# Team766/ros_vision

Hardware: AMD Instinct MI355X
Metric: frames/sec + p50 per-frame latency, 1280x720 AprilTag detect at 1/2/4/8 MI355X (higher is better)
Workload: dtype u8

## Files before the change

ros_vision_amd/csrc/at_common.h:

```cpp
#pragma once

#include <hip/hip_runtime.h>
#include <stdint.h>

#include "at_detmath.h"

namespace at {

template <int TW>
struct CclTile {
  static constexpr int W = TW, H = 32;
  static constexpr int BW = TW / 2, BH = H / 2;
  static constexpr int NT = BW * BH;
  static constexpr int NODES = 3 * NT;
  static constexpr int ROW_NODES = 3 * BW;
};
constexpr int kCclTileH = 32;
constexpr int kCclTileNodesMax = CclTile<64>::NODES;
constexpr int kHashSlots = 4096;
constexpr int kHashBits = 12;
constexpr int kPairEntCap = 65536;
constexpr int kBndRows = 4;
constexpr int kBndPts = 64 * 4 * kBndRows * 4;
constexpr int kBndStage = 1024;
constexpr int kLdsPairSlots = 512;
constexpr uint32_t kTileNarrow = 0x80000000u;
constexpr int kMaxTilesPerFrame = 1024;
constexpr int kMaxCclTiles = 1024;
struct CclDesc {
  static constexpr int Tthr = 0, Bthr = 16, Lthr = 32, Rthr = 40;
  static constexpr int TsF = 48, TsL = 64, TsR = 80, BsF = 96, BsL = 112, BsR = 128;
  static constexpr int LsF = 144, LsL = 152, RsF = 160, RsR = 168;
  static constexpr int kWords = 176;
};
constexpr int kMergeCapMax = 15360;
constexpr int kMergeLdsMax = kMergeCapMax * 10;
constexpr int kMaxPairs = 4096;
constexpr int kSortCap = 8192;
constexpr int kBlobThreads = 256;
constexpr int kWideBlobMaxBatch = 8;
constexpr int kSmallBlob = 512;
constexpr int kNMaxima = 10;
constexpr int kMaxRefineSamples = 1536;
#ifndef AT_LDS_REFINE
#define AT_LDS_REFINE 256
#endif
constexpr int kLdsRefine = AT_LDS_REFINE;
constexpr int kDecodeGridPerBlobWg = 8;
inline int decode_grid(int nblobwg, int B) {
  const int hi = nblobwg * kDecodeGridPerBlobWg, want = 64 * B;
  return nblobwg * 2 > (want < hi ? want : hi) ? nblobwg * 2 : (want < hi ? want : hi);
}

constexpr int kNumStages = 12;
constexpr const char* kStageNames[kNumStages] = {"k_pre",   "k_thr_ccl", "k_ccl_merge", "k_ccl_roots",
                                                 "k_boundary", "k_pairs", "k_group",     "k_extents",
                                                 "k_blob_small", "k_blob", "k_decode",   "k_pose"};

constexpr int kNumCls = 7;
constexpr int kNumLargeCls = 3;

constexpr uint32_t kStatusPairsOverflow = 1u;
constexpr uint32_t kStatusHashFull = 2u;
constexpr uint32_t kStatusDetsOverflow = 4u;
constexpr uint32_t kStatusPointsOverflow = 8u;
constexpr uint32_t kStatusQuadsOverflow = 16u;
constexpr uint32_t kStatusPairsCapped = 32u;
constexpr int kMaxBatch = 256;
constexpr int kQcStride = 32;
constexpr int kQuadCandPerFrame = kMaxPairs;
constexpr int kMaxDets = kQuadCandPerFrame;
constexpr int kDetPoolPerFrame = 128;
constexpr int kMaxCodes = 1024;
constexpr int kMaxFamilyBits = 64;

struct FamilyDesc {
  int nbits;
  int width_at_border;
  int total_width;
  int reversed_border;
  int ncodes;
  int8_t bitx[kMaxFamilyBits], bity[kMaxFamilyBits];
};

struct Geom {
  int W, H, Wd, Hd;
  int TW, TH;
  int BW, BH;
  int CTX, CTY;
  int ctw;
  int merge_cap;
  int merge_lds;
  int nlarge;
  int bnd_region;
  int cap_pts;
  int BTX, BTY, ntb;
  uint32_t min_cluster;
  uint32_t max_cluster;
  int min_tag_width;
};

struct Params {
  int min_white_black_diff;
  float max_line_fit_mse;
  double cos_critical_rad;
  double decode_sharpening;
  int refine_edges;
  double fx, fy, cx, cy, k1, k2, p1, p2, k3;
  int diag_stop;
  double tag_size;
  int probe;
  int taps;
  int wide_blob;
  int pipe_stop;
  int lblob_wg;
  int sblob_wg;
  int dec_wg;
  FamilyDesc fam;
  int gp_w, gp_h, gp_c;
};
constexpr int kProbeWords = 256;

#ifdef AT_EXPERIMENTS
#define AT_DIAG_STOP(prm, n) ((prm).diag_stop == (n))
#define AT_PIPE_STOP(prm) ((prm).pipe_stop)
#define AT_PROBE_ON(prm) ((prm).probe != 0)
#define AT_DIAG_ANY(prm) ((prm).diag_stop != 0)
#else
#define AT_DIAG_STOP(prm, n) false
#define AT_PIPE_STOP(prm) 0
#define AT_PROBE_ON(prm) false
#define AT_DIAG_ANY(prm) false
#endif

struct KernelTimer {
  int stage;
  hipEvent_t t0, t1;
  hipError_t (*split)(void* ctx, int which);
  void* ctx;
};

struct DevDetection {
  int32_t id;
  int16_t hamming;
  uint16_t frame;
  float decision_margin;
  int32_t blob_rank;
  double H[9];
  double c[2];
  double p[4][2];
  double pose_R[9];
  double pose_t[3];
  double pose_err[2];
};

struct QuadCand {
  uint32_t frame, rank;
  float p[4][2];
};

struct QuadRecord {
  uint32_t blob_index, valid, accepted;
  uint16_t indices[4];
  float corners[4][2];
};

struct Moments {
  int32_t Mx, My, W;
  int64_t Mxx, Myy, Mxy;
  int32_t N;
};

struct QuadPend {
  float fit[4][4];
  uint32_t blob_index, valid;
  uint16_t indices[4];
};
static_assert(sizeof(QuadPend) == 80, "QuadPend: 80 B per kept blob");

struct DrawPrim {
  double x0, y0, x1, y1;
  uint8_t bgr[3];
};

struct DevBufs {
  const uint8_t* const* frames;
  uint8_t* gray;
  uint8_t* dec;
  uint8_t* mm;
  uint8_t* thr;
  uint32_t* par;
  uint32_t* lroot;
  uint32_t* nlroot;
  uint32_t* lcnt;
  uint32_t* cdesc;
  uint32_t* ccl_ovf;
  uint32_t* nlr_tot;
  uint32_t* size;
  uint64_t* pts;
  uint32_t* tcnt;
  uint32_t* tent;
  uint32_t* grp;
  uint64_t* keys;
  uint64_t* pent_key;
  uint32_t* pent_cnt;
  uint64_t* povf_key;
  uint32_t* povf_cnt;
  uint32_t* npent;
  uint64_t* ht_key;
  uint32_t* ht_cnt;
  uint32_t* ht_rank;
  uint32_t* ht_off;
  uint32_t* ht_cur;
  uint32_t* pair_cnt;
  uint32_t* pair_off;
  uint32_t* pair_sel;
  uint32_t* work;
  uint32_t wcap;
  DevDetection* dets;
  uint32_t* det_work;
  uint32_t* det_head;
  uint32_t* dec_done;
  DevDetection* hdets;
  uint32_t* hctrl;
  uint32_t* ctrl;
  uint32_t ctrl_words;
  QuadRecord* quads;
  QuadPend* qpend;
  uint32_t* npts;
  uint32_t* npairs;
  uint32_t* ndets;
  uint32_t* nquads;
  uint32_t* status;
  uint32_t* ncls;
  uint32_t* workhead;
  uint64_t* probe;
  uint32_t* blob_pts;
  uint32_t* workhead_small;
  uint32_t* workhead_mid;
  uint32_t* nqcand;
  uint32_t qc_words;
  uint32_t* qhead;
  QuadCand* qcand;
  uint32_t qcand_cap;
  double* rsamp;
  const uint64_t* book_code;
  const int32_t* book_id;
  float* gp_out;
  int32_t kt_stage;
  uint64_t* kstamp;
  uint32_t* kgrid;
  uint64_t* kwg;
  uint32_t kwg_cap;
  uint64_t* s_pk;
};

}
```

ros_vision_amd/csrc/at_kernels.hip:

```cpp
#include <limits>
#include <hip/hip_runtime.h>

#include <float.h>
#include <math.h>
#include <stdint.h>

#include "at_common.h"
#include "at_mjpg.h"
#include "at_pose.h"


namespace at {

__device__ __forceinline__ uint32_t lane_id() { return __lane_id(); }
__device__ __attribute__((noinline)) float det_atan2f_call(float y, float x) { return det_atan2f(y, x); }

__device__ __forceinline__ uint64_t mix_hash(uint64_t k) {
  return (k * 0x9E3779B97F4A7C15ull) >> (64 - kHashBits);
}

__device__ __forceinline__ int dx_of(int dxy) { return dxy == 3 ? -1 : (dxy == 2 ? 0 : 1); }
__device__ __forceinline__ int dy_of(int dxy) { return dxy == 0 ? 0 : 1; }

template <int CTRL, int ROW_MASK, typename T>
// ... 930 lines not shown
      if (old == ka) return;
      a = (uint32_t)old;
    }
  }
}

template <int TWD>
__global__ __launch_bounds__(1024) void k_ccl_merge(DevBufs b, Geom g, Params prm) {
  using CT = CclTile<TWD>;
  constexpr int kBW = CT::BW, kBH = CT::BH;
  extern __shared__ uint64_t s_key[];
  uint16_t* s_tile = nullptr;
  uint32_t* s_cnt = nullptr;
  __shared__ uint32_t s_base[kMaxCclTiles + 1];
  __shared__ uint32_t s_wsum[16];
  const int f = blockIdx.x;
  const int tid = threadIdx.x;
  kt_begin(b, 2);
  auto stamp = [&](int k) {
    if (AT_PROBE_ON(prm) && f == 0 && tid == 0) b.probe[40 + k] = wall_clock64();
  };
  stamp(0);
  const int ntl = g.CTX * g.CTY;
  const size_t fo = (size_t)f * g.Wd * g.Hd;
  uint32_t* par = b.par + fo;
  uint32_t* size = b.size + fo;
  const uint32_t* lroot = b.lroot + (size_t)f * ntl * kCclTileNodesMax;
  const uint32_t nt = tid < ntl ? b.nlroot[(size_t)f * ntl + tid] : 0u;
  uint32_t total = 0;
  const uint32_t incl = block_incl_scan(nt, s_wsum, &total, 16);
  if (tid < ntl) s_base[tid] = incl - nt;
  if (tid == 0) {
    s_base[ntl] = total;
    b.nlr_tot[f] = total;
  }
  const bool fits = total <= (uint32_t)g.merge_cap;
  const bool cnt_lds = (size_t)total * 12 + 4 <= (size_t)g.merge_lds;
  s_tile = reinterpret_cast<uint16_t*>(s_key + total);
  s_cnt = reinterpret_cast<uint32_t*>(s_key + total);
  __syncthreads();
  if (fits && !cnt_lds)
    for (int t = tid >> 6; t < ntl; t += 16) {
      const uint32_t b0 = s_base[t], n = s_base[t + 1] - b0;
      for (uint32_t k = lane_id(); k < n; k += 64) s_tile[b0 + k] = (uint16_t)t;
    }
  __syncthreads();
  if (!fits) {
    for (int t = tid >> 6; t < ntl; t += 16) {
      const uint32_t n = s_base[t + 1] - s_base[t];
      for (uint32_t k = lane_id(); k < n; k += 64) {
        const uint32_t l = lroot[(size_t)t * kCclTileNodesMax + k];
        par[l] = l;
        size[l] = lcnt_of(b, f, ntl, t, k);
      }
    }
    if (tid == 0) b.ccl_ovf[f] = 1u;
    __threadfence();
    __syncthreads();
    constexpr int kNR = BorderRoles<TWD>::NT;
    for (int j = tid; j < ntl * kNR; j += 1024) {
      const int t = j / kNR;
      border_candidate<TWD>(b, g, f, t % g.CTX, t / g.CTX, j % kNR);
    }
    __threadfence();
    __syncthreads();
    for (int t = tid >> 6; t < ntl; t += 16) {
      const uint32_t n = s_base[t + 1] - s_base[t];
      for (uint32_t k = lane_id(); k < n; k += 64) {
        const uint32_t l = lroot[(size_t)t * kCclTileNodesMax + k];
        const uint32_t r = g_find(par, l);
        if (r != l) {
          par[l] = r;
          atomicAdd(size + r, lcnt_of(b, f, ntl, t, k));
        }
      }
    }
    __threadfence();
    __syncthreads();
    for (int t = tid >> 6; t < ntl; t += 16) {
      const uint32_t n = s_base[t + 1] - s_base[t];
      for (uint32_t k = lane_id(); k < n; k += 64) {
        const uint32_t l = lroot[(size_t)t * kCclTileNodesMax + k];
        const uint32_t r = g_load(par + l);
        par[l] = r | (g_load(size + r) >= 25 ? kKeptBit : 0u);
      }
    }
    if (b.kt_stage == 2) {
      __syncthreads();
      if (tid == 0) kt_end(b, 2);
    }
    return;
  }
  stamp(1);
  const uint32_t* lcnt = b.lcnt + (size_t)f * ntl * kCclTileNodesMax;
  uint32_t mg[kMergePer];
  if (cnt_lds) {
    for (int t = tid >> 6; t < ntl; t += 16) {
      const uint32_t b0 = s_base[t], n = s_base[t + 1] - b0;
      for (uint32_t k = lane_id(); k < n; k += 64) {
        const size_t e = (size_t)t * kCclTileNodesMax + k;
        s_cnt[b0 + k] = lcnt[e];
        s_key[b0 + k] = ((uint64_t)lroot[e] << 32) | (b0 + k);
      }
    }
  } else {
#pragma unroll
    for (int j = 0; j < kMergePer; j++) {
      const uint32_t i = tid + 1024u * j;
      mg[j] = 0;
      if (i < total) {
        const int t = s_tile[i];
        const size_t e = (size_t)t * kCclTileNodesMax + (i - s_base[t]);
        mg[j] = lroot[e];
        s_key[i] = ((uint64_t)mg[j] << 32) | i;
        size[mg[j]] = lcnt[e];
      }
    }
    __threadfence();
  }
  __syncthreads();
  stamp(2);
  const uint32_t* desc = b.cdesc + (size_t)f * ntl * CclDesc::kWords;
  auto dbyte = [&](int t, int w, int i) -> uint32_t {
    return (uint32_t)reinterpret_cast<const uint8_t*>(desc + (size_t)t * CclDesc::kWords + w)[i];
  };
  auto dslot = [&](int t, int w, int i) -> uint32_t {
    return (uint32_t)reinterpret_cast<const uint16_t*>(desc + (size_t)t * CclDesc::kWords + w)[i];
  };
  const int n0 = ntl * kBW, n1 = n0 + ntl * kBH, nitems = n1 + ntl * (kBH - 1);
  const size_t lused = (cnt_lds ? (size_t)total * 12 : (size_t)total * 10) + 7 & ~(size_t)7;
  const bool ulist = fits && lused + (size_t)16 * kMergeList * 8 <= (size_t)g.merge_lds;
  uint32_t* wl = reinterpret_cast<uint32_t*>(reinterpret_cast<uint8_t*>(s_key) + lused) + (tid >> 6) * (2 * kMergeList);
  const uint32_t wlane = lane_id();
  uint32_t nl = 0;
  auto lflush = [&]() {
    wave_sync();
    for (uint32_t i = wlane; i < nl; i += 64) merge_union(s_key, wl[2 * i], wl[2 * i + 1]);
    wave_sync();
    nl = 0;
  };
  for (int j0 = 0; j0 < nitems; j0 += 1024 * kMergeItems) {
    uint32_t su[kMergeItems][5], sv[kMergeItems][5];
#pragma unroll
    for (int q = 0; q < kMergeItems; q++) {
#pragma unroll
      for (int k = 0; k < 5; k++) su[q][k] = sv[q][k] = 0xffffffffu;
      const int j = j0 + tid + 1024 * q;
      if (j >= nitems) continue;
      if (j < n0) {
        const int t = j / kBW, x = j % kBW, ty = t / g.CTX, tx = t % g.CTX;
        if (ty == 0 || tx * kBW + x >= g.BW) continue;
        const int ta = t - g.CTX;
        const bool hl = tx > 0, hr = tx + 1 < g.CTX;
        const uint32_t a = dbyte(t, CclDesc::Tthr, 2 * x), bb = dbyte(t, CclDesc::Tthr, 2 * x + 1);
        const uint32_t ul = x > 0 ? dbyte(ta, CclDesc::Bthr, 2 * x - 1) : (hl ? dbyte(ta - 1, CclDesc::Bthr, 2 * kBW - 1) : 127u);
        const uint32_t u0 = dbyte(ta, CclDesc::Bthr, 2 * x), u1 = dbyte(ta, CclDesc::Bthr, 2 * x + 1);
        const uint32_t ur = x + 1 < kBW ? dbyte(ta, CclDesc::Bthr, 2 * x + 2) : (hr ? dbyte(ta + 1, CclDesc::Bthr, 0) : 127u);
        const uint32_t bF = s_base[t], bA = s_base[ta];
        const uint32_t oF = dslot(t, CclDesc::TsF, x), oL = dslot(t, CclDesc::TsL, x), oR = dslot(t, CclDesc::TsR, x);
        if (a == 255 && ul == 255) {
          const int tv = x > 0 ? ta : ta - 1;
          su[q][0] = bF + oF;
          sv[q][0] = s_base[tv] + dslot(tv, CclDesc::BsF, x > 0 ? x - 1 : kBW - 1);
        }
        if ((a == 255 || bb == 255) && (u0 == 255 || u1 == 255)) {
          su[q][1] = bF + oF;
          sv[q][1] = bA + dslot(ta, CclDesc::BsF, x);
        }
        if (bb == 255 && ur == 255) {
          const int tv = x + 1 < kBW ? ta : ta + 1;
          su[q][2] = bF + oF;
          sv[q][2] = s_base[tv] + dslot(tv, CclDesc::BsF, x + 1 < kBW ? x + 1 : 0);
        }
        if (a == 0 && u0 == 0) { su[q][3] = bF + oL; sv[q][3] = bA + dslot(ta, CclDesc::BsL, x); }
        if (bb == 0 && u1 == 0) { su[q][4] = bF + oR; sv[q][4] = bA + dslot(ta, CclDesc::BsR, x); }
      } else if (j < n1) {
        const int t = (j - n0) / kBH, y = (j - n0) % kBH, ty = t / g.CTX, tx = t % g.CTX;
        if (tx == 0 || ty * kBH + y >= g.BH) continue;
        const int tl = t - 1;
        const uint32_t a = dbyte(t, CclDesc::Lthr, 2 * y), c = dbyte(t, CclDesc::Lthr, 2 * y + 1);
        const uint32_t ul = y > 0 ? dbyte(tl, CclDesc::Rthr, 2 * y - 1) : 127u;
        const uint32_t l0 = dbyte(tl, CclDesc::Rthr, 2 * y), l1 = dbyte(tl, CclDesc::Rthr, 2 * y + 1);
        const uint32_t bF = s_base[t], bL = s_base[tl];
        const uint32_t oF = dslot(t, CclDesc::LsF, y), oL = dslot(t, CclDesc::LsL, y);
        if (y > 0 && a == 255 && ul == 255) { su[q][0] = bF + oF; sv[q][0] = bL + dslot(tl, CclDesc::RsF, y - 1); }
        if ((a == 255 || c == 255) && (l0 == 255 || l1 == 255)) { su[q][1] = bF + oF; sv[q][1] = bL + dslot(tl, CclDesc::RsF, y); }
        if ((a == 0 && l0 == 0) || (c == 0 && l1 == 0)) { su[q][2] = bF + oL; sv[q][2] = bL + dslot(tl, CclDesc::RsR, y); }
      } else {
        const int t = (j - n1) / (kBH - 1), y = 1 + (j - n1) % (kBH - 1), ty = t / g.CTX, tx = t % g.CTX;
        if ((tx + 1) * kBW > g.BW || ty * kBH + y >= g.BH || tx + 1 >= g.CTX) continue;
        const uint32_t bb = dbyte(t, CclDesc::Rthr, 2 * y), ur = dbyte(t + 1, CclDesc::Lthr, 2 * y - 1);
        if (bb == 255 && ur == 255) {
          su[q][0] = s_base[t] + dslot(t, CclDesc::RsF, y);
          sv[q][0] = s_base[t + 1] + dslot(t + 1, CclDesc::LsF, y - 1);
        }
      }
    }
#pragma unroll
    for (int q = 0; q < kMergeItems; q++)
#pragma unroll
      for (int k = 0; k < 5; k++) {
        const bool on = su[q][k] != 0xffffffffu && sv[q][k] < (uint32_t)total && su[q][k] < (uint32_t)total;
        const uint32_t pair = on ? (su[q][k] << 16 | sv[q][k]) : 0xffffffffu;
        const uint32_t prev = wave_shr1(pair, 0xfffffffeu);
        if (ulist) {
          const bool act = on && pair != prev;
          const uint64_t m = __ballot(act);
          const uint32_t c = (uint32_t)__popcll(m);
          if (nl + c > (uint32_t)kMergeList) lflush();
          if (act) {
            const uint32_t pos = nl + lanes_below(m);
            wl[2 * pos] = su[q][k];
            wl[2 * pos + 1] = sv[q][k];
          }
          nl += c;
          continue;
        }
        if (on && pair != prev) merge_union(s_key, su[q][k], sv[q][k]);
      }
  }
  if (ulist && nl) lflush();
  __syncthreads();
  stamp(3);
#pragma unroll
  for (int j = 0; j < kMergePer; j++) {
    const uint32_t i = tid + 1024u * j;
    if (i < total) {
      const uint32_t r = merge_find(s_key, i);
      if (r != i) {
        if (cnt_lds) {
          atomicAdd(&s_cnt[r], s_cnt[i]);
        } else {
          const int t = s_tile[i];
          atomicAdd(size + (uint32_t)(key_load(s_key + r) >> 32), lcnt[(size_t)t * kCclTileNodesMax + (i - s_base[t])]);
        }
      }
    }
  }
  if (!cnt_lds) __threadfence();
  __syncthreads();
  stamp(4);
  if (cnt_lds) {
    for (int t = tid >> 6; t < ntl; t += 16) {
      const uint32_t b0 = s_base[t], n = s_base[t + 1] - b0;
      for (uint32_t k = lane_id(); k < n; k += 64) {
        const uint32_t node = lroot[(size_t)t * kCclTileNodesMax + k];
        const uint32_t i = b0 + k;
        const uint32_t r = merge_find(s_key, i);
        const uint32_t root = (uint32_t)(key_load(s_key + r) >> 32);
        const uint32_t cnt = s_cnt[r];
        par[node] = root | (cnt >= 25 ? kKeptBit : 0u);
        if (prm.taps && r == i) size[node] = cnt;
      }
    }
  } else {
#pragma unroll
    for (int j = 0; j < kMergePer; j++) {
      const uint32_t i = tid + 1024u * j;
      if (i < total) {
        const uint32_t r = merge_find(s_key, i);
        const uint32_t root = (uint32_t)(key_load(s_key + r) >> 32);
        par[mg[j]] = root | (g_load(size + root) >= 25 ? kKeptBit : 0u);
      }
    }
  }
  stamp(5);
  if (b.kt_stage == 2) {
    __syncthreads();
    if (tid == 0) kt_end(b, 2);
  }
}

__device__ __forceinline__ uint64_t make_qbp(uint32_t rep0, uint32_t rep1, uint32_t x, uint32_t y, int dxy,
                                             bool b2w) {
  const uint32_t lo = rep0 < rep1 ? rep0 : rep1, hi = rep0 < rep1 ? rep1 : rep0;
  return ((uint64_t)(hi & 0xfffff) << 44) | ((uint64_t)(lo & 0xfffff) << 24) | ((uint64_t)(x & 0x3ff) << 14) |
         ((uint64_t)(y & 0x3ff) << 4) | ((uint64_t)(b2w ? 1 : 0) << 3) | (uint64_t)(dxy & 3);
}

__device__ uint32_t ht_slot_find(const uint64_t* keys, uint64_t key) {
  uint32_t s = (uint32_t)mix_hash(key);
  for (int probe = 0; probe < kHashSlots; probe++) {
    const uint64_t k = keys[s];
    if (k == key) return s;
    if (k == 0) return 0xffffffffu;
    s = (s + 1) & (kHashSlots - 1);
  }
  return 0xffffffffu;
}

__device__ __forceinline__ uint64_t wave_shr1_u64(uint64_t v) {
  return (uint64_t)wave_shr1((uint32_t)v, 0) | ((uint64_t)wave_shr1((uint32_t)(v >> 32), 0) << 32);
}


#ifndef AT_BND_HASH32
#define AT_BND_HASH32 1
#endif
__device__ __forceinline__ uint32_t pair_hash(uint64_t key) {
  static_assert(kLdsPairSlots == 512, "9-bit slot hash");
  if (AT_BND_HASH32) return ((uint32_t)key * 0x9E3779B1u) >> 23;
  return (uint32_t)(mix_hash(key) & (kLdsPairSlots - 1));
}
__device__ __forceinline__ bool lds_pair_add(uint64_t* keys, uint32_t* cnts, uint64_t key, uint32_t len) {
  uint32_t h = pair_hash(key);
  for (int probe = 0; probe < kLdsPairSlots; probe++) {
    const uint64_t k = keys[h];
    if (k == key) {
      atomicAdd(cnts + h, len);
      return true;
    }
    if (k == 0) {
      const uint64_t prev = atomicCAS((unsigned long long*)(keys + h), 0ull, (unsigned long long)key);
      if (prev == 0 || prev == key) {
        atomicAdd(cnts + h, len);
        return true;
      }
    }
    h = (h + 1) & (kLdsPairSlots - 1);
  }
  return false;
}

__device__ __forceinline__ uint32_t lds_pair_slot(const uint64_t* keys, uint64_t key) {
  uint32_t h = pair_hash(key);
  while (keys[h] != key) h = (h + 1) & (kLdsPairSlots - 1);
  return h;
}

__device__ __forceinline__ uint32_t narrow_point(uint32_t entry, uint64_t key) {
  return (entry << 23) | ((uint32_t)(key >> 1) & 0x7ffffcu) | ((uint32_t)key & 3u);
}
__device__ __forceinline__ uint32_t narrow_bits(uint32_t w) { return ((w & 0x7ffffcu) << 1) | (w & 3u); }


__device__ __forceinline__ void bnd_spill(const DevBufs& b, int f, uint64_t key, uint32_t cnt) {
  const uint32_t o = atomicAdd(b.npent + f, 1u);
  if (o < (uint32_t)kPairEntCap) {
    b.povf_key[(size_t)f * kPairEntCap + o] = key;
    b.povf_cnt[(size_t)f * kPairEntCap + o] = cnt;
  } else {
    atomicOr(b.status + f, kStatusHashFull);
  }
}

#ifdef AT_BND_SGPRS
#define AT_BND_ATTR __attribute__((amdgpu_num_sgpr(AT_BND_SGPRS)))
#else
#define AT_BND_ATTR
#endif
template <bool KEPT>
__global__ __launch_bounds__(256) AT_BND_ATTR void k_boundary(DevBufs b, Geom g) {
  __shared__ uint64_t s_pkey[kLdsPairSlots];
  __shared__ uint32_t s_pcnt[kLdsPairSlots];
  __shared__ uint64_t s_pts[kBndStage];
  __shared__ uint32_t s_npts, s_nent, s_spill;
  __shared__ __attribute__((aligned(4))) uint8_t s_tthr[(4 * kBndRows + 1) * 66];
  __shared__ uint32_t s_tlab[(4 * kBndRows + 1) * 66];
  const TileIdx bi = xcd_block<AT_XCD_BND>();
  const int f = bi.z;
  const int tid = threadIdx.y * 64 + threadIdx.x;
  kt_begin(b, 4);
  for (int i = tid; i < kLdsPairSlots; i += 256) {
    s_pkey[i] = 0;
    s_pcnt[i] = 0;
  }
  if (tid == 0) { s_npts = 0; s_nent = 0; s_spill = 0; }
  const size_t fo = (size_t)f * g.Wd * g.Hd;
  const uint8_t* thr = b.thr + fo;
  const uint32_t* par = b.par + fo;
  const int Wd = g.Wd;
  const int ty0 = 1 + bi.y * (4 * kBndRows), tx0 = bi.x * 64;
  constexpr int kTR = 4 * kBndRows + 1, kTC = 66, kTN = kTR * kTC;
  constexpr int kPer = (kTN + 255) / 256;
  uint32_t lv[kPer], lb[kPer];
  uint8_t tv[kPer];
#pragma unroll
  for (int k = 0; k < kPer; k++) {
    const int e = tid + 256 * k, ec = min(e, kTN - 1);
    const int yy = ty0 + ec / kTC, xx = tx0 + ec % kTC;
    const bool in = e < kTN && yy < g.Hd && xx < Wd;
    const int yc = min(yy, g.Hd - 1), xc = min(xx, Wd - 1);
    const uint32_t F = node_F(g, yc >> 1, xc >> 1), LR = node_L(g, yc >> 1, 0) + (uint32_t)xc;
    const uint8_t t = thr[(size_t)yc * Wd + xc];
    const uint32_t a = par[F], c = par[LR];
    tv[k] = in ? t : (uint8_t)127;
    lv[k] = in ? a : 0xffffffffu;
    lb[k] = in ? c : 0xffffffffu;
  }
#pragma unroll
  for (int k = 0; k < kPer; k++) {
    lv[k] = tv[k] == 127 ? 0xffffffffu : (tv[k] == 255 ? lv[k] : lb[k]);
    const uint32_t r = par[lv[k] != 0xffffffffu ? (lv[k] & ~kKeptBit) : 0u];
    lv[k] = lv[k] != 0xffffffffu ? r : 0xffffffffu;
  }
#pragma unroll
  for (int k = 0; k < kPer; k++) {
    const int e = tid + 256 * k;
    if (e < kTN) {
      const bool kept = lv[k] != 0xffffffffu && (KEPT ? (lv[k] & kKeptBit) != 0 : b.size[fo + lv[k]] >= 25);
      s_tlab[e] = lv[k] & ~kKeptBit;
      s_tthr[e] = kept ? tv[k] : (uint8_t)127;
    }
  }
  __syncthreads();
  const uint32_t lane = lane_id();
  const size_t tb = (size_t)f * g.ntb + bi.y * gridDim.x + bi.x;
  uint64_t* pts_out = b.pts + tb * g.bnd_region;
  const int cx = 2 * (int)(lane & 31);
  const int xa = 1 + bi.x * 64 + cx;
  for (int r = 0; r < kBndRows / 2; r++) {
    const int ly = (r * 4 + threadIdx.y) * 2 + (int)(lane >> 5);
    const int y = ty0 + ly;
    const int eb = ly * kTC + cx;
    const uint32_t ra = (uint32_t)*reinterpret_cast<const uint16_t*>(s_tthr + eb) |
                        ((uint32_t)*reinterpret_cast<const uint16_t*>(s_tthr + eb + 2) << 16);
    const uint32_t rb = (uint32_t)*reinterpret_cast<const uint16_t*>(s_tthr + eb + kTC) |
                        ((uint32_t)*reinterpret_cast<const uint16_t*>(s_tthr + eb + kTC + 2) << 16);
    uint32_t hm = 0, nb[8], rep[2];
    bool b2w[2];
#pragma unroll
    for (int j = 0; j < 2; j++) {
      rep[j] = 0;
      b2w[j] = false;
#pragma unroll
      for (int d = 0; d < 4; d++) nb[4 * j + d] = 0;
      const uint32_t v0 = (ra >> (8 * j + 8)) & 0xff;
      const uint32_t vl = (ra >> (8 * j)) & 0xff, vr = (ra >> (8 * j + 16)) & 0xff;
      const uint32_t vdl = (rb >> (8 * j)) & 0xff, vd = (rb >> (8 * j + 8)) & 0xff, vdr = (rb >> (8 * j + 16)) & 0xff;
      const int e0 = eb + j + 1, ed = e0 + kTC;
      const bool pv = xa + j <= g.Wd - 2 && y <= g.Hd - 2 && v0 != 127;
      rep[j] = s_tlab[e0];
      b2w[j] = v0 == 0;
      nb[4 * j] = s_tlab[e0 + 1];
      nb[4 * j + 1] = s_tlab[ed + 1];
      nb[4 * j + 2] = s_tlab[ed];
      nb[4 * j + 3] = s_tlab[ed - 1];
      const bool dedup = vl != 127 && vd != 127 && vd != vl && xa + j != 1;
      const uint32_t pm = (v0 + vr == 255 ? 1u : 0u) | (v0 + vdr == 255 ? 2u : 0u) | (v0 + vd == 255 ? 4u : 0u) |
                          (!dedup && v0 + vdl == 255 ? 8u : 0u);
      hm |= pv ? pm << (4 * j) : 0u;
    }
    const bool got = hm != 0;
    const uint32_t rf = (hm & 0xfu) ? rep[0] : rep[1];
    uint32_t nf = nb[7];
#pragma unroll
    for (int d = 6; d >= 0; d--) nf = ((hm >> d) & 1) ? nb[d] : nf;
    uint32_t cnt = 0, xm = 0;
#pragma unroll
    for (int d = 0; d < 8; d++) {
      const uint32_t rj = rep[d >> 2];
      const bool in = (hm >> d) & 1, eq = (rj == rf && nb[d] == nf) || (rj == nf && nb[d] == rf);
      cnt += in && eq;
      xm |= (in && !eq) ? 1u << d : 0u;
    }
    const uint32_t npts = (uint32_t)__builtin_popcount(hm);
    const uint32_t sc = wave_incl_scan(cnt | (npts << 16), AddOp(), 0u);
    const uint32_t incl = sc & 0xffffu;
    const uint32_t below = (sc >> 16) - npts, wtot = wave_read(sc, 63) >> 16;
    const uint64_t kp = got ? make_qbp(rf, nf, 0, 0, 0, false) >> 24 : 0ull;
    {
      const uint64_t prev = wave_shr1_u64(kp);
      const bool same = got && lane > 0 && prev == kp;
      const uint64_t same_mask = __ballot(same);
      const bool head = got && !same;
      const uint32_t len = head ? run_len(same_mask, lane) : 1u;
      const uint32_t incl_end = (uint32_t)__shfl((int)incl, (int)(lane + len - 1));
      if (head) {
        const uint32_t tot = incl_end - incl + cnt;
        if (!lds_pair_add(s_pkey, s_pcnt, kp, tot)) {
          bnd_spill(b, f, kp, tot);
          s_spill = 1;
        }
      }
      if (__ballot(xm != 0)) {
#pragma unroll
        for (int d = 0; d < 8; d++) {
          if ((xm >> d) & 1) {
            const uint64_t k = make_qbp(rep[d >> 2], nb[d], 0, 0, 0, false) >> 24;
            if (!lds_pair_add(s_pkey, s_pcnt, k, 1u)) {
              bnd_spill(b, f, k, 1u);
              s_spill = 1;
            }
          }
        }
      }
    }
    uint32_t wbase = 0;
    if (lane == 0 && wtot) wbase = atomicAdd(&s_npts, wtot);
    wbase = __shfl(wbase, 0);
    uint32_t pos = wbase + below;
    if (wbase + wtot <= (uint32_t)kBndStage) {
#pragma unroll
      for (int d = 0; d < 8; d++)
        if ((hm >> d) & 1) s_pts[pos++] = make_qbp(rep[d >> 2], nb[d], xa + (d >> 2), y, d & 3, b2w[d >> 2]);
    } else {
#pragma unroll
      for (int d = 0; d < 8; d++)
        if ((hm >> d) & 1) {
          const uint64_t k = make_qbp(rep[d >> 2], nb[d], xa + (d >> 2), y, d & 3, b2w[d >> 2]);
          if (pos < (uint32_t)kBndStage) s_pts[pos] = k;
          else if (pos < (uint32_t)g.bnd_region) pts_out[pos] = k;
          else atomicOr(b.status + f, kStatusPointsOverflow);
          pos++;
        }
    }
  }
  __syncthreads();
  const uint32_t total = s_npts;
  const bool narrow = total <= (uint32_t)kBndStage && !s_spill;
  uint64_t* ekey = b.pent_key + tb * kLdsPairSlots;
  uint32_t* ecnt = b.pent_cnt + tb * kLdsPairSlots;
  uint32_t* s_ent = s_tlab;
  for (int i = tid; i < kLdsPairSlots; i += 256) {
    const uint64_t k = s_pkey[i];
    if (k) {
      const uint32_t o = atomicAdd(&s_nent, 1u);
      ekey[o] = k;
      ecnt[o] = s_pcnt[i];
      s_ent[i] = o;
    }
  }
  if (narrow) {
    __syncthreads();
    uint32_t* out = reinterpret_cast<uint32_t*>(pts_out);
    for (uint32_t i = tid; i < total; i += 256) {
      const uint64_t k = s_pts[i];
      out[i] = narrow_point(s_ent[lds_pair_slot(s_pkey, k >> 24)], k);
    }
  } else {
    const uint32_t staged = total < (uint32_t)kBndStage ? total : (uint32_t)kBndStage;
    for (uint32_t i = tid; i < staged; i += 256) pts_out[i] = s_pts[i];
  }
  __syncthreads();
  if (tid == 0) {
    b.tcnt[tb] = min(total, (uint32_t)g.bnd_region) | (narrow ? kTileNarrow : 0u);
    b.tent[tb] = s_nent;
    kt_end(b, 4);
  }
}

__device__ __forceinline__ int size_class(uint32_t n) {
  if (n > 2048) return 0;
  if (n > 1024) return 1;
  if (n > (uint32_t)kSmallBlob) return 2;
  if (n > 256) return 3;
  if (n > 128) return 4;
  if (n > 64) return 5;
  return 6;
}

template <typename T, int NT>
__device__ void block_bitonic_sort(T* s, int n) {
  for (int k = 2; k <= n; k <<= 1) {
    for (int j = k >> 1; j > 0; j >>= 1) {
      for (int i = threadIdx.x; i < n; i += NT) {
        const int ixj = i ^ j;
        if (ixj > i) {
          const T a = s[i], c = s[ixj];
          const bool up = (i & k) == 0;
          if ((a > c) == up) {
            s[i] = c;
            s[ixj] = a;
          }
        }
      }
      __syncthreads();
    }
  }
}

constexpr int kGrpEnt = 128;
constexpr uint32_t kGrpDrop = 0xfffffffeu, kGrpFallback = 0xffffffffu;
constexpr int kPairsEntCache = 4;

__global__ __launch_bounds__(1024) void k_pairs(DevBufs b, Geom g, int probe) {
  const int f = blockIdx.x;
  const int tid = threadIdx.x;
  auto stamp = [&](int i) {
    if (probe && f == 0 && tid == 0) b.probe[i] = wall_clock64();
  };
  stamp(0);
  __shared__ uint64_t t_key[kHashSlots];
  __shared__ uint32_t t_cnt[kHashSlots];
  uint64_t* s_list = t_key;
  static_assert(kMaxPairs <= kHashSlots, "the pair list fits in the hash table's storage");
  __shared__ uint32_t s_n, s_full, s_np;
  __shared__ uint32_t s_wsum[16];
  for (int i = tid; i < kHashSlots; i += 1024) {
    t_key[i] = 0;
    t_cnt[i] = 0;
  }
  if (tid == 0) { s_n = 0; s_full = 0; s_np = 0; }
  __syncthreads();
  auto merge = [&](uint64_t key, uint32_t cnt) -> uint32_t {
    uint32_t h = (uint32_t)mix_hash(key) & (kHashSlots - 1);
    for (int probe = 0; probe < kHashSlots; probe++) {
      const uint64_t k = t_key[h];
      if (k == key) {
        atomicAdd(&t_cnt[h], cnt);
        return h;
      } else if (k == 0) {
        const uint64_t prev = atomicCAS((unsigned long long*)&t_key[h], 0ull, (unsigned long long)key);
        if (prev == 0 || prev == key) {
          atomicAdd(&t_cnt[h], cnt);
          return h;
        }
      }
      h = (h + 1) & (kHashSlots - 1);
    }
    s_full = 1;
    return 0xffffffffu;
  };
  uint32_t c_slot[kPairsEntCache], c_cnt[kPairsEntCache], c_idx[kPairsEntCache];
  bool c_lds[kPairsEntCache];
  __shared__ uint32_t s_tpre[kMaxTilesPerFrame + 1];
  uint32_t tot_e = 0;
  const int ntb = g.ntb;
  uint32_t novf = 0;
  {
    const uint32_t ne = tid < ntb ? b.tent[(size_t)f * ntb + tid] : 0u;
    const uint32_t np = tid < ntb ? b.tcnt[(size_t)f * ntb + tid] & ~kTileNarrow : 0u;
    const uint32_t incl_e = block_incl_scan(ne, s_wsum, &tot_e, 16);
    if (tid < ntb) s_tpre[tid] = incl_e - ne;
    if (tid == 0) s_tpre[ntb] = tot_e;
    if (np) atomicAdd(&s_np, np);
    novf = min(b.npent[f], (uint32_t)kPairEntCap);
    __syncthreads();
  }
  auto entry = [&](uint32_t i, uint32_t* et) -> size_t {
    int lo = 0, hi = ntb - 1;
    while (lo < hi) {
      const int mid = (lo + hi + 1) >> 1;
      if (s_tpre[mid] <= i) lo = mid;
      else hi = mid - 1;
    }
    *et = i - s_tpre[lo];
    return ((size_t)f * ntb + lo) * kLdsPairSlots + *et;
  };
  auto merge_pass = [&](uint64_t limit) {
#pragma unroll
    for (int k = 0; k < kPairsEntCache; k++) { c_slot[k] = 0xffffffffu; c_cnt[k] = 0; c_idx[k] = 0; c_lds[k] = false; }
    {
      uint32_t et[kPairsEntCache], cnt[kPairsEntCache];
      uint64_t key[kPairsEntCache];
      size_t e[kPairsEntCache];
#pragma unroll
      for (int k = 0; k < kPairsEntCache; k++) {
        const uint32_t i = tid + 1024u * k;
        e[k] = i < tot_e ? entry(i, &et[k]) : 0;
      }
#pragma unroll
      for (int k = 0; k < kPairsEntCache; k++) {
        const bool in = tid + 1024u * k < tot_e;
        cnt[k] = in ? b.pent_cnt[e[k]] : 0u;
        key[k] = in ? b.pent_key[e[k]] : 0ull;
      }
#pragma unroll
      for (int k = 0; k < kPairsEntCache; k++) {
        if (tid + 1024u * k >= tot_e) continue;
        c_slot[k] = key[k] < limit ? merge(key[k], cnt[k]) : 0xffffffffu;
        c_cnt[k] = cnt[k];
        c_idx[k] = (uint32_t)e[k];
        c_lds[k] = et[k] < (uint32_t)kGrpEnt;
      }
    }
    for (uint32_t i = tid + 1024u * kPairsEntCache; i < tot_e; i += 1024) {
      uint32_t et;
      const size_t e = entry(i, &et);
      const uint64_t key = b.pent_key[e];
      if (key < limit) merge(key, b.pent_cnt[e]);
    }
    for (uint32_t i = tid; i < novf; i += 1024) {
      const uint64_t key = b.povf_key[(size_t)f * kPairEntCap + i];
      if (key < limit) merge(key, b.povf_cnt[(size_t)f * kPairEntCap + i]);
    }
    __syncthreads();
  };
  merge_pass(~0ull);
  bool capped = false;
  if (s_full) {
    capped = true;
    uint64_t lo = 0, hi = 1ull << 40;
    while (hi - lo > 1) {
      const uint64_t mid = lo + ((hi - lo) >> 1);
      for (int i = tid; i < kHashSlots; i += 1024) { t_key[i] = 0; t_cnt[i] = 0; }
      if (tid == 0) s_full = 0;
      __syncthreads();
      for (uint32_t i = tid; i < tot_e; i += 1024) {
        uint32_t et;
        const uint64_t key = b.pent_key[entry(i, &et)];
        if (key < mid && !s_full) merge(key, 1u);
      }
      for (uint32_t i = tid; i < novf; i += 1024) {
        const uint64_t key = b.povf_key[(size_t)f * kPairEntCap + i];
        if (key < mid && !s_full) merge(key, 1u);
      }
      __syncthreads();
      const bool ok = !s_full;
      __syncthreads();
      if (ok) lo = mid;
      else hi = mid;
    }
    for (int i = tid; i < kHashSlots; i += 1024) { t_key[i] = 0; t_cnt[i] = 0; }
    if (tid == 0) s_full = 0;
    __syncthreads();
    merge_pass(lo);
  }
  for (uint32_t i = tid + 1024 * kPairsEntCache; i < tot_e; i += 1024) {
    uint32_t et;
    const size_t e = entry(i, &et);
    if (et < (uint32_t)kGrpEnt) b.pent_cnt[e] = kGrpFallback;
  }
  __syncthreads();
  if (tid == 0) {
    b.npts[f] = s_np;
    b.npent[f] = tot_e + novf;
    if (capped) atomicOr(b.status + f, kStatusPairsCapped);
  }
  __syncthreads();
  stamp(1);
  static_assert(kHashSlots == 4 * 1024, "four hash slots per thread");
  uint64_t kreg[4];
#pragma unroll
  for (int k = 0; k < 4; k++) {
    const int s = tid + 1024 * k;
    kreg[k] = t_key[s];
    b.ht_key[(size_t)f * kHashSlots + s] = kreg[k];
    b.ht_cnt[(size_t)f * kHashSlots + s] = t_cnt[s];
  }
  __syncthreads();
#pragma unroll
  for (int k = 0; k < 4; k++) {
    if (kreg[k]) {
      const uint32_t i = atomicAdd(&s_n, 1u);
      if (i < kMaxPairs) s_list[i] = (kreg[k] << kHashBits) | (uint64_t)(tid + 1024 * k);
    }
  }
  __syncthreads();
  const uint32_t n = s_n;
  if (tid == 0) b.npairs[f] = n;
  if (n > (uint32_t)kMaxPairs || s_full) {
    if (tid == 0) atomicOr(b.status + f, s_full ? kStatusHashFull : kStatusPairsOverflow);
    return;
  }
  int np2 = 64;
  while (np2 < (int)n) np2 <<= 1;
  for (int i = (int)n + tid; i < np2; i += 1024) s_list[i] = ~0ull;
  __syncthreads();
  stamp(2);
  if (n <= 1024) {
    const int P = (int)(1024 / (n ? n : 1u));
    uint32_t* s_rank = reinterpret_cast<uint32_t*>(t_key + 2048);
    if (tid < (int)n) s_rank[tid] = 0;
    __syncthreads();
    if (tid < P * (int)n) {
      const int i = tid % (int)n, h = tid / (int)n;
      const uint64_t key = s_list[i];
      const int j1 = (int)(((uint32_t)h + 1) * n / (uint32_t)P);
      int j = (int)((uint32_t)h * n / (uint32_t)P);
      uint32_t r = 0;
      for (; j + 4 <= j1; j += 4)
        r += (s_list[j] < key) + (s_list[j + 1] < key) + (s_list[j + 2] < key) + (s_list[j + 3] < key);
      for (; j < j1; j++) r += s_list[j] < key;
      if (r) atomicAdd(&s_rank[i], r);
    }
    __syncthreads();
    if (tid < (int)n) t_key[1024 + s_rank[tid]] = s_list[tid];
    __syncthreads();
    if (tid < (int)n) s_list[tid] = t_key[1024 + tid];
    __syncthreads();
  } else {
    block_bitonic_sort<uint64_t, 1024>(s_list, np2);
  }
  stamp(3);
  const int i0 = tid * 4;
  uint32_t lslt[4];
#pragma unroll
  for (int k = 0; k < 4; k++) lslt[k] = i0 + k < (int)n ? (uint32_t)(s_list[i0 + k] & (kHashSlots - 1)) : 0u;
  auto cnt_at = [&](int k) -> uint32_t { return i0 + k < (int)n ? t_cnt[lslt[k]] : 0u; };
  const uint32_t c0 = cnt_at(0), c1 = cnt_at(1), c2 = cnt_at(2), c3 = cnt_at(3);
  const uint32_t tsum = c0 + c1 + c2 + c3;
  const uint32_t incl = wave_incl_scan(tsum, AddOp(), 0u);
  const uint32_t lane = lane_id();
  if (lane == 63) s_wsum[tid >> 6] = incl;
  __syncthreads();
  uint32_t wbase = 0;
  for (int w = 0; w < (tid >> 6); w++) wbase += s_wsum[w];
  const uint32_t excl = wbase + incl - tsum;
  const uint32_t offs[4] = {excl, excl + c0, excl + c0 + c1, excl + c0 + c1 + c2};
  const uint32_t cs[4] = {c0, c1, c2, c3};
  stamp(4);
  __shared__ uint32_t s_ccnt[kNumCls], s_cbase[kNumCls];
  __syncthreads();
  if (tid < kNumCls) s_ccnt[tid] = 0;
  __syncthreads();
  int cls[4];
  uint32_t lslot[4];
#pragma unroll
  for (int k = 0; k < 4; k++) {
    cls[k] = -1;
    lslot[k] = 0;
    if (i0 + k < (int)n && cs[k] >= g.min_cluster && cs[k] <= g.max_cluster) {
      cls[k] = size_class(cs[k]);
      lslot[k] = atomicAdd(&s_ccnt[cls[k]], 1u);
    }
  }
  __syncthreads();
  if (tid < kNumCls) s_cbase[tid] = s_ccnt[tid] ? atomicAdd(b.ncls + tid, s_ccnt[tid]) : 0u;
  __syncthreads();
#pragma unroll
  for (int k = 0; k < 4; k++) {
    const int i = i0 + k;
    if (i < (int)n) {
      const uint32_t slot = lslt[k];
      b.ht_rank[(size_t)f * kHashSlots + slot] = (uint32_t)i;
      b.ht_off[(size_t)f * kHashSlots + slot] = offs[k];
      b.pair_cnt[(size_t)f * kMaxPairs + i] = cs[k];
      b.pair_off[(size_t)f * kMaxPairs + i] = offs[k];
      b.pair_sel[(size_t)f * kMaxPairs + i] = 0;
      if (cls[k] >= 0)
        b.work[(size_t)cls[k] * b.wcap + s_cbase[cls[k]] + lslot[k]] = ((uint32_t)f << 16) | (uint32_t)i;
    }
  }
  uint32_t* t_off = reinterpret_cast<uint32_t*>(t_key);
  uint32_t* t_cur = t_off + kHashSlots;
#pragma unroll
  for (int k = 0; k < 4; k++) {
    const int i = i0 + k;
    if (i < (int)n) {
      const uint32_t slot = lslt[k];
      t_off[slot] = offs[k];
      t_cur[slot] = 0;
    }
  }
// ... 3131 lines not shown
```

Measured before the change: 141,400.

## Stage boundary points as 32-bit slot-encoded words and recompute wide points on spill

lds_pair_add now returns the hash slot, which is broadcast to each run's lanes, so staged boundary points are stored in LDS as 32-bit words (slot, x, y, direction). The final pass then remaps them with a direct table lookup instead of re-probing the hash per point. Halving the per-point size lets the staging buffer double to 2048 entries in the same LDS space, so more tiles stay on the narrow path. When a tile overflows or spills, the points are recomputed and written as 64-bit keys straight to global memory. This adds a second pass for those tiles and relies on the x/y bit packing staying consistent with what downstream consumers expect.

```diff
diff --git a/ros_vision_amd/csrc/at_common.h b/ros_vision_amd/csrc/at_common.h
--- a/ros_vision_amd/csrc/at_common.h
+++ b/ros_vision_amd/csrc/at_common.h
@@ -22,7 +22,7 @@
 constexpr int kPairEntCap = 65536;
 constexpr int kBndRows = 4;
 constexpr int kBndPts = 64 * 4 * kBndRows * 4;
-constexpr int kBndStage = 1024;
+constexpr int kBndStage = 2048;
 constexpr int kLdsPairSlots = 512;
 constexpr uint32_t kTileNarrow = 0x80000000u;
 constexpr int kMaxTilesPerFrame = 1024;
diff --git a/ros_vision_amd/csrc/at_kernels.hip b/ros_vision_amd/csrc/at_kernels.hip
--- a/ros_vision_amd/csrc/at_kernels.hip
+++ b/ros_vision_amd/csrc/at_kernels.hip
@@ -1256,35 +1256,28 @@
   if (AT_BND_HASH32) return ((uint32_t)key * 0x9E3779B1u) >> 23;
   return (uint32_t)(mix_hash(key) & (kLdsPairSlots - 1));
 }
-__device__ __forceinline__ bool lds_pair_add(uint64_t* keys, uint32_t* cnts, uint64_t key, uint32_t len) {
+constexpr uint32_t kNoPairSlot = 0xffffffffu;
+__device__ __forceinline__ uint32_t lds_pair_add(uint64_t* keys, uint32_t* cnts, uint64_t key, uint32_t len) {
   uint32_t h = pair_hash(key);
   for (int probe = 0; probe < kLdsPairSlots; probe++) {
     const uint64_t k = keys[h];
     if (k == key) {
       atomicAdd(cnts + h, len);
-      return true;
+      return h;
     }
     if (k == 0) {
       const uint64_t prev = atomicCAS((unsigned long long*)(keys + h), 0ull, (unsigned long long)key);
       if (prev == 0 || prev == key) {
         atomicAdd(cnts + h, len);
-        return true;
+        return h;
       }
     }
     h = (h + 1) & (kLdsPairSlots - 1);
   }
-  return false;
-}
-
-__device__ __forceinline__ uint32_t lds_pair_slot(const uint64_t* keys, uint64_t key) {
-  uint32_t h = pair_hash(key);
-  while (keys[h] != key) h = (h + 1) & (kLdsPairSlots - 1);
-  return h;
-}
-
-__device__ __forceinline__ uint32_t narrow_point(uint32_t entry, uint64_t key) {
-  return (entry << 23) | ((uint32_t)(key >> 1) & 0x7ffffcu) | ((uint32_t)key & 3u);
-}
+  return kNoPairSlot;
+}
+
+__device__ __forceinline__ uint32_t narrow_xy(uint32_t x, uint32_t y) { return ((x & 0x3ff) << 13) | ((y & 0x3ff) << 3); }
 __device__ __forceinline__ uint32_t narrow_bits(uint32_t w) { return ((w & 0x7ffffcu) << 1) | (w & 3u); }
 
 
@@ -1307,7 +1300,7 @@
 __global__ __launch_bounds__(256) AT_BND_ATTR void k_boundary(DevBufs b, Geom g) {
   __shared__ uint64_t s_pkey[kLdsPairSlots];
   __shared__ uint32_t s_pcnt[kLdsPairSlots];
-  __shared__ uint64_t s_pts[kBndStage];
+  __shared__ uint32_t s_pts[kBndStage];
   __shared__ uint32_t s_npts, s_nent, s_spill;
   __shared__ __attribute__((aligned(4))) uint8_t s_tthr[(4 * kBndRows + 1) * 66];
   __shared__ uint32_t s_tlab[(4 * kBndRows + 1) * 66];
@@ -1363,16 +1356,16 @@
   uint64_t* pts_out = b.pts + tb * g.bnd_region;
   const int cx = 2 * (int)(lane & 31);
   const int xa = 1 + bi.x * 64 + cx;
-  for (int r = 0; r < kBndRows / 2; r++) {
-    const int ly = (r * 4 + threadIdx.y) * 2 + (int)(lane >> 5);
+  auto step_points = [&](int r, int wrow, uint32_t lane, int cx, int xa, uint32_t& hm, uint32_t (&nb)[8], uint32_t (&rep)[2],
+                         bool (&b2w)[2]) {
+    const int ly = (r * 4 + wrow) * 2 + (int)(lane >> 5);
     const int y = ty0 + ly;
     const int eb = ly * kTC + cx;
     const uint32_t ra = (uint32_t)*reinterpret_cast<const uint16_t*>(s_tthr + eb) |
                         ((uint32_t)*reinterpret_cast<const uint16_t*>(s_tthr + eb + 2) << 16);
     const uint32_t rb = (uint32_t)*reinterpret_cast<const uint16_t*>(s_tthr + eb + kTC) |
                         ((uint32_t)*reinterpret_cast<const uint16_t*>(s_tthr + eb + kTC + 2) << 16);
-    uint32_t hm = 0, nb[8], rep[2];
-    bool b2w[2];
+    hm = 0;
 #pragma unroll
     for (int j = 0; j < 2; j++) {
       rep[j] = 0;
@@ -1395,6 +1388,12 @@
                           (!dedup && v0 + vdl == 255 ? 8u : 0u);
       hm |= pv ? pm << (4 * j) : 0u;
     }
+    return y;
+  };
+  for (int r = 0; r < kBndRows / 2; r++) {
+    uint32_t hm, nb[8], rep[2];
+    bool b2w[2];
+    const int y = step_points(r, (int)threadIdx.y, lane, cx, xa, hm, nb, rep, b2w);
     const bool got = hm != 0;
     const uint32_t rf = (hm & 0xfu) ? rep[0] : rep[1];
     uint32_t nf = nb[7];
@@ -1413,56 +1412,86 @@
     const uint32_t incl = sc & 0xffffu;
     const uint32_t below = (sc >> 16) - npts, wtot = wave_read(sc, 63) >> 16;
     const uint64_t kp = got ? make_qbp(rf, nf, 0, 0, 0, false) >> 24 : 0ull;
-    {
-      const uint64_t prev = wave_shr1_u64(kp);
-      const bool same = got && lane > 0 && prev == kp;
-      const uint64_t same_mask = __ballot(same);
-      const bool head = got && !same;
-      const uint32_t len = head ? run_len(same_mask, lane) : 1u;
-      const uint32_t incl_end = (uint32_t)__shfl((int)incl, (int)(lane + len - 1));
-      if (head) {
-        const uint32_t tot = incl_end - incl + cnt;
-        if (!lds_pair_add(s_pkey, s_pcnt, kp, tot)) {
-          bnd_spill(b, f, kp, tot);
-          s_spill = 1;
-        }
-      }
-      if (__ballot(xm != 0)) {
-#pragma unroll
-        for (int d = 0; d < 8; d++) {
-          if ((xm >> d) & 1) {
-            const uint64_t k = make_qbp(rep[d >> 2], nb[d], 0, 0, 0, false) >> 24;
-            if (!lds_pair_add(s_pkey, s_pcnt, k, 1u)) {
-              bnd_spill(b, f, k, 1u);
-              s_spill = 1;
-            }
-          }
-        }
-      }
-    }
+    const uint64_t prev = wave_shr1_u64(kp);
+    const bool same = got && lane > 0 && prev == kp;
+    const uint64_t same_mask = __ballot(same);
+    const bool head = got && !same;
+    const uint32_t len = head ? run_len(same_mask, lane) : 1u;
+    const uint32_t incl_end = (uint32_t)__shfl((int)incl, (int)(lane + len - 1));
+    uint32_t slot = kNoPairSlot;
+    if (head) {
+      const uint32_t tot = incl_end - incl + cnt;
+      slot = lds_pair_add(s_pkey, s_pcnt, kp, tot);
+      if (slot == kNoPairSlot) {
+        bnd_spill(b, f, kp, tot);
+        s_spill = 1;
+      }
+    }
+    const uint64_t hb = __ballot(head) << (63 - lane);
+    slot = (uint32_t)__shfl((int)slot, hb ? (int)lane - __builtin_clzll(hb) : (int)lane);
     uint32_t wbase = 0;
     if (lane == 0 && wtot) wbase = atomicAdd(&s_npts, wtot);
     wbase = __shfl(wbase, 0);
-    uint32_t pos = wbase + below;
-    if (wbase + wtot <= (uint32_t)kBndStage) {
+    const uint32_t pos0 = wbase + below;
+    const bool fits = wbase + wtot <= (uint32_t)kBndStage;
+    const uint32_t wxy = narrow_xy(xa, y);
+    if (fits) {
+      uint32_t pos = pos0;
+      const uint32_t w0 = (slot << 23) | wxy;
 #pragma unroll
       for (int d = 0; d < 8; d++)
-        if ((hm >> d) & 1) s_pts[pos++] = make_qbp(rep[d >> 2], nb[d], xa + (d >> 2), y, d & 3, b2w[d >> 2]);
-    } else {
+        if ((hm >> d) & 1) s_pts[pos++] = (w0 + ((uint32_t)(d >> 2) << 13)) | (b2w[d >> 2] ? 4u : 0u) | (uint32_t)(d & 3);
+    }
+    if (__ballot(xm != 0)) {
+#pragma unroll
+      for (int d = 0; d < 8; d++) {
+        if ((xm >> d) & 1) {
+          int e0 = (y - ty0) * kTC + cx + 1 + (d >> 2);
+          asm volatile("" : "+v"(e0));
+          const int en = e0 + ((d & 3) == 0 ? 1 : (d & 3) == 1 ? kTC + 1 : (d & 3) == 2 ? kTC : kTC - 1);
+          const uint64_t k = make_qbp(s_tlab[e0], s_tlab[en], 0, 0, 0, false) >> 24;
+          const uint32_t sx = lds_pair_add(s_pkey, s_pcnt, k, 1u);
+          if (sx == kNoPairSlot) {
+            bnd_spill(b, f, k, 1u);
+            s_spill = 1;
+          } else if (fits) {
+            s_pts[pos0 + (uint32_t)__builtin_popcount(hm & ((1u << d) - 1u))] =
+                (((sx << 23) | wxy) + ((uint32_t)(d >> 2) << 13)) | (b2w[d >> 2] ? 4u : 0u) | (uint32_t)(d & 3);
+          }
+        }
+      }
+    }
+  }
+  __syncthreads();
+  const uint32_t total = s_npts;
+  const bool narrow = total <= (uint32_t)kBndStage && !s_spill;
+  if (!narrow) {
+    uint32_t wl = threadIdx.x, wt = threadIdx.y;
+    asm volatile("" : "+v"(wl), "+v"(wt));
+    const int wcx = 2 * (int)(wl & 31), wxa = 1 + bi.x * 64 + wcx;
+    for (int r = 0; r < kBndRows / 2; r++) {
+      uint32_t hm, nb[8], rep[2];
+      bool b2w[2];
+      const int y = step_points(r, (int)wt, wl, wcx, wxa, hm, nb, rep, b2w);
+      const uint32_t npts = (uint32_t)__builtin_popcount(hm);
+      const uint32_t sc = wave_incl_scan(npts, AddOp(), 0u);
+      const uint32_t wtot = wave_read(sc, 63);
+      uint32_t wbase = 0;
+      if (wl == 0 && wtot) wbase = atomicAdd(&s_nent, wtot);
+      wbase = __shfl(wbase, 0);
+      uint32_t pos = wbase + sc - npts;
 #pragma unroll
       for (int d = 0; d < 8; d++)
         if ((hm >> d) & 1) {
-          const uint64_t k = make_qbp(rep[d >> 2], nb[d], xa + (d >> 2), y, d & 3, b2w[d >> 2]);
-          if (pos < (uint32_t)kBndStage) s_pts[pos] = k;
-          else if (pos < (uint32_t)g.bnd_region) pts_out[pos] = k;
+          if (pos < (uint32_t)g.bnd_region) pts_out[pos] = make_qbp(rep[d >> 2], nb[d], wxa + (d >> 2), y, d & 3, b2w[d >> 2]);
           else atomicOr(b.status + f, kStatusPointsOverflow);
           pos++;
         }
     }
-  }
-  __syncthreads();
-  const uint32_t total = s_npts;
-  const bool narrow = total <= (uint32_t)kBndStage && !s_spill;
+    __syncthreads();
+    if (tid == 0) s_nent = 0;
+    __syncthreads();
+  }
   uint64_t* ekey = b.pent_key + tb * kLdsPairSlots;
   uint32_t* ecnt = b.pent_cnt + tb * kLdsPairSlots;
   uint32_t* s_ent = s_tlab;
@@ -1479,12 +1508,9 @@
     __syncthreads();
     uint32_t* out = reinterpret_cast<uint32_t*>(pts_out);
     for (uint32_t i = tid; i < total; i += 256) {
-      const uint64_t k = s_pts[i];
-      out[i] = narrow_point(s_ent[lds_pair_slot(s_pkey, k >> 24)], k);
-    }
-  } else {
-    const uint32_t staged = total < (uint32_t)kBndStage ? total : (uint32_t)kBndStage;
-    for (uint32_t i = tid; i < staged; i += 256) pts_out[i] = s_pts[i];
+      const uint32_t w = s_pts[i];
+      out[i] = (s_ent[w >> 23] << 23) | (w & 0x7fffffu);
+    }
   }
   __syncthreads();
   if (tid == 0) {
```

After: 143,300, median of 6. +1.3%, better.
